# TrondVQ/UncertaintyQuantification-SleepApnea-1DCNN

Hardware: AMD Instinct MI355X
Metric: 30s-windows/sec for MCD T=50 & DE M=8 inference at 1/2/4/8 MI355X (higher is better)
Workload: dtype fp32; 1 GPU; global_batch=16384, seq_len=60, parallelism=dp1, mcd_passes=50, de_members=8, bn_mode_mcd=batch

## Files before the change

uncertaintyquantification_sleepapnea_1dcnn_amd/csrc/x3_dense_map.h:

```cpp
#pragma once

#ifndef __host__
#define APNEAUQ_X3_DENSE_MAP_PLAIN 1
#define __host__
#define __device__
#endif

namespace apneauq {
namespace x3 {
namespace dense {

constexpr int kLen = 60, kSlot = 64, kHaloRows = 4;

__host__ __device__ constexpr long long tiles(long long n_win, int rows) { return (kLen * n_win + rows - 1) / rows; }
__host__ __device__ constexpr int max_windows(int rows) { return (kLen - 4 + rows - 1) / kLen + 1; }
__host__ __device__ constexpr int lds_rows(int rows) { return kHaloRows + kSlot * max_windows(rows) + kHaloRows; }

__host__ __device__ constexpr long long first_row(long long tl, int rows) { return tl * rows; }
__host__ __device__ constexpr int first_window(long long tl, int rows) { return (int)(first_row(tl, rows) / kLen); }
__host__ __device__ constexpr int offset(long long tl, int rows) { return (int)(first_row(tl, rows) % kLen); }
__host__ __device__ constexpr int windows(int off, int rows) { return (off + rows - 1) / kLen + 1; }

__host__ __device__ constexpr int slot_of(int dl) { return (int)(((unsigned)dl & 1023u) * 1093u >> 16); }
__host__ __device__ constexpr int step_of(int dl) { return dl - kLen * slot_of(dl); }
__host__ __device__ constexpr int lds_row(int dl) { return kHaloRows + dl + (kSlot - kLen) * slot_of(dl); }

__host__ __device__ constexpr int staged_units(int rows, int pad) { return rows + 2 * pad; }
__host__ __device__ constexpr bool staged(int dl, int off, int rows, int pad) {
  return dl >= 0 && dl >= off - pad && dl < off + rows + pad && dl < kLen * windows(off, rows);
}

}
}
}

#ifdef APNEAUQ_X3_DENSE_MAP_PLAIN
#undef __host__
#undef __device__
#undef APNEAUQ_X3_DENSE_MAP_PLAIN
#endif
```

uncertaintyquantification_sleepapnea_1dcnn_amd/csrc/x3_layers.hip:

```cpp
#include "common.h"
#include "x3_args.h"
#include "x3_dense_map.h"

namespace apneauq {
namespace x3 {

typedef _Float16 f16x8 __attribute__((ext_vector_type(8)));
typedef _Float16 f16x4 __attribute__((ext_vector_type(4)));
typedef _Float16 f16x2 __attribute__((ext_vector_type(2)));
typedef __attribute__((address_space(1))) const f16x8 gf16x8;

constexpr int kStagers = 4;
constexpr int kL = 60, kSR = 64, kHalo = 4;
__host__ __device__ constexpr int row_bytes(int ck) { return 4 * ck + 32; }
__device__ __forceinline__ int sample_prescale(unsigned rmax_bits, const float* amax) {
  const float b = __builtin_fmaf(amax[0], __uint_as_float(rmax_bits), amax[1]);
  int e = 0;
  if (b > 0.f && b < INFINITY) frexpf(b, &e);
  return min(100, max(-100, 14 - e));
}

__host__ __device__ constexpr int lds_rows(int S) { return kHalo + S * kSR + kHalo; }
__host__ __device__ constexpr int buf_bytes(int S, int ck) { return lds_rows(S) * row_bytes(ck); }
__host__ __device__ constexpr int lds_bytes(int S, int cout, int ck, bool dense_rows = false) {
  return 2 * (dense_rows ? dense::lds_rows(kSR * S) * row_bytes(ck) : buf_bytes(S, ck)) + 2 * cout * 8 + 2 * S * 4;
}

template <typename T>
__device__ __forceinline__ T gld(const void* p) {
  return *(const __attribute__((address_space(1))) T*)(p);
}

__device__ __forceinline__ int opaque_tid() {
  int t = threadIdx.x;
  asm volatile("" : "+v"(t));
  return t;
}

__device__ __forceinline__ f32x4 mfma(const f16x8& a, const f16x8& b, const f32x4& c) {
  return __builtin_amdgcn_mfma_f32_16x16x32_f16(a, b, c, 0, 0, 0);
}

__device__ __forceinline__ void lds_barrier() {
  __builtin_amdgcn_fence(__ATOMIC_RELEASE, "workgroup", "local");
  __builtin_amdgcn_s_barrier();
  __builtin_amdgcn_fence(__ATOMIC_ACQUIRE, "workgroup", "local");
}

__device__ __forceinline__ int xcd_wg() {
  const int nwg = gridDim.x, bid = blockIdx.x;
  const int q = nwg / 8, rem = nwg % 8, xcd = bid % 8;
  return (xcd < rem ? xcd * (q + 1) : rem * (q + 1) + (xcd - rem) * q) + bid / 8;
}

template <int NW, int WPC>
constexpr int waves_per_eu() { return NW * WPC > 8 ? (NW * WPC + 3) / 4 : NW * WPC <= 4 ? 1 : 2; }
constexpr int loaders(int lw) { return lw > 0 ? lw : 0; }
template <int CIN, int COUT, int KS, int S, int WM, int WN, bool LAST, int LW, int CK, int WPC, bool PS, bool DENSE = false>
__global__ __launch_bounds__((WM * WN + loaders(LW)) * 64, (waves_per_eu<WM * WN + loaders(LW), WPC>())) void layer_kernel(
    const LayerArgs A) {
  extern __shared__ __attribute__((aligned(16))) char smem[];
  constexpr int NWM = WM * WN, NW = NWM + loaders(LW), kThreads = NW * 64;
  constexpr int kCK = CK, kRowB = row_bytes(CK), NQ = CK / 32, kQ = CK / 4;
  constexpr int PAD = (KS - 1) / 2, kRows = kSR * S;
  static_assert(!DENSE || (!PS && !LAST), "dense rows: batch-moment blocks 2..5 only");
  constexpr int kS = S, kBufB = DENSE ? dense::lds_rows(kRows) * kRowB : buf_bytes(S, CK);
  constexpr int kValidRows = DENSE ? kRows : S * kL, kUnits = kValidRows * kQ;
  constexpr int SW = LW > 0 ? LW : LW < 0 ? (-LW < NW ? -LW : NW) : (kStagers < NW ? kStagers : NW);
  constexpr int kSBase = LW > 0 ? NWM * 64 : 0;
  constexpr int kST = SW * 64;
  constexpr int kMainU = (kUnits + kST - 1) / kST, kNU = kMainU + (DENSE ? 1 : 0);
  constexpr int kEdgeWaves = (2 * PAD * kQ + 63) / 64;
  static_assert(!DENSE || (kUnits % kST == 0 && kEdgeWaves <= SW), "dense rows: whole staging steps per tile");
  static_assert(kST % kQ == 0 && (CK == 32 || CK == 64), "a staging thread keeps one channel quad");
  constexpr int NCH = CIN / kCK, NCTA = COUT / 16, NCT = NCTA / WN, NRT = 4 * S / WM;
  constexpr int NSTEP = NCH * NQ * KS;
  constexpr int RG = NCT >= 4                        ? 1
                     : (NCT >= 3 && NCT * NRT > 16)    ? 1
                     : NCT == 1                        ? 4
                                                       : 2;
  constexpr bool BDB = NCT * NRT <= 24 && RG < 4;
  static_assert(NRT % RG == 0, "row-tile groups");
  constexpr long long FRAG_STEP = (long long)NCTA * 128;
  static_assert(CIN % kCK == 0 && COUT % 16 == 0, "channel tiling");
  static_assert(NCTA % WN == 0 && (4 * S) % WM == 0, "wave tiling");
  static_assert(NRT % 4 == 0, "whole 64-row sample slots per wave row (epilogue keys, block 6 sums)");
  double* st = reinterpret_cast<double*>(smem + 2 * kBufB);
  float* wsc = reinterpret_cast<float*>(smem + 2 * kBufB + 2 * COUT * 8);

  const int tid = threadIdx.x, lane = tid & 63;
  const int wave = __builtin_amdgcn_readfirstlane(tid >> 6);
  const int wn = wave % WN, wm = (wave / WN) % WM;
  const int ct0 = wn * NCT, rt0 = wm * NRT;
  const int m = lane & 15, h = lane >> 4;
  APNEAUQ_DASSERT(blockDim.x == kThreads);

  for (int i = tid; i < 2 * kBufB / 16; i += kThreads) reinterpret_cast<f32x4*>(smem)[i] = f32x4{0.f, 0.f, 0.f, 0.f};
  for (int i = tid; i < 2 * COUT; i += kThreads) st[i] = 0.0;
  __syncthreads();

  const int wg = xcd_wg();
  const int tpg = DENSE ? (int)dense::tiles(A.n_win, kRows) : (A.n_win + S - 1) / S;
  const int total_tiles = tpg * A.groups;
  const int t_begin = (int)((long long)wg * total_tiles / gridDim.x);
  const int t_end = (int)((long long)(wg + 1) * total_tiles / gridDim.x);
  if (t_begin >= t_end) return;
  const int slot = wg % kStatSlots;

  const bool loader = LW > 0 && wave >= NWM;
  const bool stager = LW > 0 ? loader : wave < SW;
  const bool edge_wave = DENSE && wave >= kSBase / 64 && wave - kSBase / 64 < kEdgeWaves;
  auto dense_unit = [&](int u, int tid, int off, int& dl) -> bool {
    const int r = tid / kQ;
    if (u < kMainU) {
      dl = off + r + (kST / kQ) * u;
      return true;
    }
    dl = r < PAD ? off - PAD + r : off + kRows - PAD + r;
    return edge_wave && r < 2 * PAD && dense::staged(dl, off, kRows, PAD);
  };
  struct Stage {
    f32x4 v[kNU];
    f32x4 a, b;
  };
  Stage s0;
  const bool hash_in = A.thr_in != 0u && !A.sign_in;
  const bool sign_in = A.thr_in != 0u && A.sign_in;
  const bool prescale = PS && A.smax_in != nullptr;
  int key_tile = -1;
  unsigned skeys[kS];
  unsigned skey_tile = 0u;
  static_assert(kS <= 8, "packed per-sample exponents");
  constexpr int kSP = (kS + 3) / 4;
  unsigned sa_pack[kSP];
  auto load_chunk = [&](int tile, int c, Stage& R) {
    const int tid = opaque_tid() - kSBase, q = tid % kQ;
    const int g = tile / tpg;
    const int w0 = (tile - g * tpg) * (DENSE ? kRows : kS);
    const float* af = A.aff_in + (long long)g * A.aff_gstride + c * kCK + 4 * q;
    R.a = gld<f32x4>(af);
    R.b = gld<f32x4>(af + CIN);
#pragma unroll
    for (int u = 0; u < kNU; ++u) {
      const int ri = tid / kQ + (kST / kQ) * u;
      R.v[u] = f32x4{-0.f, -0.f, -0.f, -0.f};
      if constexpr (DENSE) {
        const int wf = w0 / kL, off = w0 - wf * kL;
        int dl;
        if (dense_unit(u, tid, off, dl) && wf + dense::slot_of(dl) < A.n_win) {
          const long long r0 = (A.in_shared ? 0ll : (long long)g * A.n_win * kL) + wf * kL;
          R.v[u] = gld<f32x4>(A.in + (r0 + dl) * CIN + c * kCK + 4 * q);
        }
      } else if (ri < kValidRows) {
        const int s = ri / kL, t = ri - s * kL, w = w0 + s;
        if (w < A.n_win) {
          const long long si = A.in_shared ? w : (long long)g * A.n_win + w;
          R.v[u] = gld<f32x4>(A.in + (si * kL + t) * CIN + c * kCK + 4 * q);
        }
      }
    }
  };
  auto store_chunk = [&](int tile, int c, char* buf, const Stage& R) {
    const int tid = opaque_tid() - kSBase, q = tid % kQ;
    const int g = tile / tpg;
    const int w0 = (tile - g * tpg) * (DENSE ? kRows : kS);
    if (tile != key_tile) {
      const unsigned skey = stream_key(A.seed, A.layer - 1, A.pass_base + g);
      skey_tile = skey;
      const float* am = A.amax_in + (A.aff_gstride ? 2 * g : 0);
      float ws0 = A.wscale[A.p_gstride ? g : 0];
      if (A.gscale_in != nullptr) ws0 *= A.gscale_in[A.aff_gstride ? g : 0];
#pragma unroll
      for (int i = 0; i < kSP; ++i) sa_pack[i] = 0u;
      if (DENSE && tid == 0) wsc[(tile & 1) * kS] = ws0;
#pragma unroll
      for (int s = 0; s < (DENSE ? 0 : kS); ++s) {
        skeys[s] = sample_key(skey, A.window_offset + w0 + s);
        int sa = 0;
        if (prescale && w0 + s < A.n_win) {
          const long long si = A.in_shared ? w0 + s : (long long)g * A.n_win + w0 + s;
          sa = sample_prescale(A.smax_in[si], am);
          sa_pack[s >> 2] |= ((unsigned)sa & 0xFFu) << (8 * (s & 3));
        }
        if (tid == s) wsc[(tile & 1) * kS + s] = ldexpf(ws0, -sa);
      }
      key_tile = tile;
    }
#pragma unroll
    for (int u = 0; u < kNU; ++u) {
      const int ri = tid / kQ + (kST / kQ) * u;
      int s, t, w, lrow;
      if constexpr (DENSE) {
        const int wf = w0 / kL, off = w0 - wf * kL;
        int dl;
        if (!dense_unit(u, tid, off, dl)) continue;
        s = dense::slot_of(dl), t = dl - s * kL, w = wf + s, lrow = dense::lds_row(dl);
      } else {
        if (ri >= kValidRows) continue;
        s = ri / kL, t = ri - s * kL, w = w0 + s, lrow = kHalo + s * kSR + t;
      }
      const f32x4 v = R.v[u];
      bool keep[4];
      if (hash_in) {
        unsigned k;
        if constexpr (!PS) {
          k = sample_key(skey_tile, A.window_offset + w);
        } else {
          k = skeys[0];
#pragma unroll
          for (int j = 1; j < kS; ++j) k = s == j ? skeys[j] : k;
        }
        const unsigned b01 = dropout_bits2(k, t, c * kCK + 4 * q);
        const unsigned b23 = dropout_bits2(k, t, c * kCK + 4 * q + 2);
        keep[0] = (b01 & 0xFFFFu) >= A.thr_in;
        keep[1] = (b01 >> 16) >= A.thr_in;
        keep[2] = (b23 & 0xFFFFu) >= A.thr_in;
        keep[3] = (b23 >> 16) >= A.thr_in;
      } else if (sign_in) {
#pragma unroll
        for (int i = 0; i < 4; ++i) keep[i] = !__builtin_signbit(v[i]);
      } else {
#pragma unroll
        for (int i = 0; i < 4; ++i) keep[i] = true;
      }
      const bool valid = w < A.n_win;
      int sa = 0;
      if (prescale) {
        unsigned sp = sa_pack[0];
#pragma unroll
        for (int i = 1; i < kSP; ++i) sp = (s >> 2) == i ? sa_pack[i] : sp;
        sa = __builtin_amdgcn_sbfe((int)sp, 8 * (s & 3), 8);
      }
      float a[4];
#pragma unroll
      for (int i = 0; i < 4; ++i) a[i] = (valid && keep[i]) ? ldexpf(__builtin_fmaf(v[i], R.a[i], R.b[i]), sa) : 0.f;
      uint2 hi, lo;
#pragma unroll
      for (int p = 0; p < 2; ++p) {
        const unsigned u = __builtin_bit_cast(unsigned, (f16x2){(_Float16)a[2 * p], (_Float16)a[2 * p + 1]});
        unsigned l;
        asm("v_fma_mixlo_f16 %0, %1, -1.0, %2 op_sel_hi:[1,0,0]" : "=v"(l) : "v"(u), "v"(a[2 * p]));
        asm("v_fma_mixhi_f16 %0, %1, -1.0, %2 op_sel:[1,0,0] op_sel_hi:[1,0,0]"
                     : "+v"(l)
                     : "v"(u), "v"(a[2 * p + 1]));
        (p ? hi.y : hi.x) = u;
        (p ? lo.y : lo.x) = l;
      }
      char* row = buf + lrow * kRowB + 8 * q;
      *reinterpret_cast<uint2*>(row) = hi;
      *reinterpret_cast<uint2*>(row + 2 * kCK) = lo;
    }
  };

  f32x4 acc[NCT][NRT];
#pragma unroll
  for (int ct = 0; ct < NCT; ++ct)
#pragma unroll
    for (int rt = 0; rt < NRT; ++rt) acc[ct][rt] = f32x4{0.f, 0.f, 0.f, 0.f};
  auto wbase = [&](int tile) -> const gf16x8* {
    const int g = tile / tpg;
    return (const gf16x8*)(A.wfrag) + (long long)g * A.w_gstride + ct0 * 128 + lane;
  };
  f16x8 ah[NCT], al[NCT];
  auto load_a = [&](const gf16x8* p, f16x8 (&xh)[NCT], f16x8 (&xl)[NCT]) {
#pragma unroll
    for (int ct = 0; ct < NCT; ++ct) {
      xh[ct] = p[ct * 128];
      xl[ct] = p[ct * 128 + 64];
    }
  };

  const int bofs = ((rt0 * 16 + m + kHalo - PAD) * kRowB) + 16 * h;

  auto compute_chunk = [&](int c, int off, const char* buf, const gf16x8* wcur, const gf16x8* wnxt, auto&& hook) {
    const char* bp[DENSE ? NRT : 1];
    if constexpr (DENSE) {
#pragma unroll
      for (int rt = 0; rt < NRT; ++rt)
        bp[rt] = buf + bofs + (off + (dense::kSlot - kL) * ((off + (rt0 + rt) * 16 + m) / kL)) * kRowB;
    }
#pragma unroll
    for (int kk = 0; kk < NQ * KS; ++kk) {
      const int q2 = kk / KS, j = kk - q2 * KS;
      const char* bb = buf + bofs + q2 * 64;
      const int s = c * NQ * KS + kk;
      const gf16x8* np = (s + 1 < NSTEP) ? wcur + (long long)(s + 1) * FRAG_STEP : wnxt;
      f16x8 nh[NCT], nl[NCT];
      load_a(np, nh, nl);
      __builtin_amdgcn_sched_barrier(0);
      auto ldb = [&](int rt, f16x8& h_, f16x8& l_) {
        const char* br = DENSE ? bp[rt] + q2 * 64 : bb;
        h_ = *reinterpret_cast<const f16x8*>(br + (rt * 16 + j) * kRowB);
        l_ = *reinterpret_cast<const f16x8*>(br + (rt * 16 + j) * kRowB + 2 * kCK);
      };
      f16x8 bh[RG], bl[RG];
#pragma unroll
      for (int r = 0; r < RG; ++r) ldb(r, bh[r], bl[r]);
#pragma unroll
      for (int rg = 0; rg < NRT; rg += RG) {
        f16x8 bh2[RG], bl2[RG];
#pragma unroll
        for (int r = 0; r < RG; ++r) {
          bh2[r] = bh[r];
          bl2[r] = bl[r];
          if (BDB && rg + RG < NRT) ldb(rg + RG + r, bh2[r], bl2[r]);
          if (!BDB) ldb(rg + r, bh[r], bl[r]);
        }
        __builtin_amdgcn_sched_barrier(0);
#pragma unroll
        for (int r = 0; r < RG; ++r)
#pragma unroll
          for (int ct = 0; ct < NCT; ++ct) acc[ct][rg + r] = mfma(ah[ct], bh[r], acc[ct][rg + r]);
#pragma unroll
        for (int r = 0; r < RG; ++r)
#pragma unroll
          for (int ct = 0; ct < NCT; ++ct) acc[ct][rg + r] = mfma(al[ct], bh[r], acc[ct][rg + r]);
#pragma unroll
        for (int r = 0; r < RG; ++r)
#pragma unroll
          for (int ct = 0; ct < NCT; ++ct) acc[ct][rg + r] = mfma(ah[ct], bl[r], acc[ct][rg + r]);
#pragma unroll
        for (int r = 0; r < RG; ++r) {
          bh[r] = bh2[r];
          bl[r] = bl2[r];
        }
      }
#pragma unroll
      for (int ct = 0; ct < NCT; ++ct) {
        ah[ct] = nh[ct];
        al[ct] = nl[ct];
      }
      __builtin_amdgcn_sched_barrier(0);
      if (kk == (NQ * KS) / 2) hook();
    }
  };

  auto epilogue = [&](int tile) {
    const int lane = opaque_tid() & 63, m = lane & 15, h = lane >> 4;
    const int g = tile / tpg;
    const int w0 = (tile - g * tpg) * (DENSE ? kRows : kS);
    float wsq[NRT / 4];
#pragma unroll
    for (int q = 0; q < NRT / 4; ++q) wsq[q] = wsc[(tile & 1) * kS + (DENSE ? 0 : (rt0 >> 2) + q)];
    const bool track = PS && !LAST && A.smax_out != nullptr;
    float mxs[NRT / 4];
#pragma unroll
    for (int q = 0; q < NRT / 4; ++q) mxs[q] = 0.f;
    const float* bias = A.bias + (long long)g * A.p_gstride;
    const bool drop = (LAST || A.sign_out) && A.thr_out != 0u;
    constexpr int NKEY = DENSE ? dense::max_windows(kRows) : NRT / 4;
    const int wf = DENSE ? w0 / kL : 0, off = DENSE ? w0 - wf * kL : 0;
    unsigned skeys[NKEY];
    if (drop) {
      const unsigned skey = stream_key(A.seed, A.layer, A.pass_base + g);
#pragma unroll
      for (int q = 0; q < NKEY; ++q)
        skeys[q] = DENSE ? __builtin_amdgcn_readfirstlane(sample_key(skey, A.window_offset + wf + q))
                         : sample_key(skey, A.window_offset + w0 + (rt0 >> 2) + q);
    }
#pragma unroll
    for (int ct = 0; ct < NCT; ++ct) {
      const int co0 = (ct0 + ct) * 16 + 4 * h;
      const f32x4 b4 = gld<f32x4>(bias + co0);
      f32x4 s1 = {0.f, 0.f, 0.f, 0.f}, s2 = s1, k1 = s1, k0 = s1;
      int mo = m;
      if constexpr (DENSE) asm volatile("" : "+v"(mo));
#pragma unroll
      for (int rt = 0; rt < NRT; ++rt) {
        int t, w, sl = 0;
        bool valid;
        if constexpr (DENSE) {
          const int dl = off + (rt0 + rt) * 16 + mo;
          sl = dense::slot_of(dl), w = wf + sl, t = dl - sl * kL, valid = w < A.n_win;
        } else {
          const int s = (rt0 + rt) >> 2;
          t = (((rt0 + rt) & 3) << 4) + m, w = w0 + s, valid = t < kL && w < A.n_win;
        }
        f32x4 r;
#pragma unroll
        for (int e = 0; e < 4; ++e) r[e] = fmaxf(__builtin_fmaf(acc[ct][rt][e], wsq[rt >> 2], b4[e]), 0.f);
        acc[ct][rt] = f32x4{0.f, 0.f, 0.f, 0.f};
        bool keep[4] = {true, true, true, true};
        if (drop) {
          unsigned key = skeys[DENSE ? 0 : rt >> 2];
          if constexpr (DENSE) {
#pragma unroll
            for (int q = 1; q < NKEY; ++q) key = sl == q ? skeys[q] : key;
          }
          const unsigned b01 = dropout_bits2(key, t, co0), b23 = dropout_bits2(key, t, co0 + 2);
          keep[0] = (b01 & 0xFFFFu) >= A.thr_out;
          keep[1] = (b01 >> 16) >= A.thr_out;
          keep[2] = (b23 & 0xFFFFu) >= A.thr_out;
          keep[3] = (b23 >> 16) >= A.thr_out;
        }
        if (valid) {
#pragma unroll
          for (int e = 0; e < 4; ++e) {
            s1[e] += r[e];
            s2[e] = __builtin_fmaf(r[e], r[e], s2[e]);
            if (!LAST) mxs[rt >> 2] = fmaxf(mxs[rt >> 2], r[e]);
            if constexpr (LAST) {
              k1[e] += keep[e] ? r[e] : 0.f;
              k0[e] += keep[e] ? 1.f : 0.f;
            }
          }
          if constexpr (!LAST) {
            const long long sample = (long long)g * A.n_win + w;
            f32x4 o = r;
            if (drop) {
#pragma unroll
              for (int e = 0; e < 4; ++e) o[e] = keep[e] ? r[e] : __builtin_copysignf(r[e], -1.f);
            }
            *reinterpret_cast<f32x4*>(A.out + (sample * kL + t) * COUT + co0) = o;
          }
        }
        if constexpr (LAST) {
          if ((rt & 3) == 3) {
#pragma unroll
            for (int e = 0; e < 4; ++e) {
              k1[e] = group16_sum(k1[e]);
              k0[e] = group16_sum(k0[e]);
            }
            const int wl = w0 + (rt0 + rt) / 4;
            if (m == 0 && wl < A.n_win) {
              float* o = A.out + ((long long)g * A.n_win + wl) * (2 * COUT);
              *reinterpret_cast<f32x4*>(o + co0) = k1;
              *reinterpret_cast<f32x4*>(o + COUT + co0) = k0;
            }
            k1 = f32x4{0.f, 0.f, 0.f, 0.f};
            k0 = k1;
          }
        }
      }
      if (A.stats != nullptr) {
#pragma unroll
        for (int e = 0; e < 4; ++e) {
          const float a = group16_sum(s1[e]), b = group16_sum(s2[e]);
          if (m == 0) {
            atomicAdd(&st[co0 + e], (double)a);
            atomicAdd(&st[COUT + co0 + e], (double)b);
          }
        }
      }
    }
    if (track) {
#pragma unroll
      for (int q = 0; q < NRT / 4; ++q) {
        const float mq = wave_max(mxs[q]);
        const int w = w0 + (rt0 >> 2) + q;
        if (lane == 0 && w < A.n_win) atomicMax(A.smax_out + (long long)g * A.n_win + w, __float_as_uint(mq));
      }
    }
  };

  auto flush_stats = [&](int g) {
    __syncthreads();
    if (A.stats != nullptr) {
      double* dst = A.stats + ((long long)g * kStatSlots + slot) * 2 * COUT;
      for (int i = tid; i < 2 * COUT; i += kThreads) {
        atomicAdd(dst + i, st[i]);
        st[i] = 0.0;
      }
    }
    __syncthreads();
  };

  const int total = (t_end - t_begin) * NCH;
  auto chunk_tile = [&](int it) { return t_begin + it / NCH; };
  auto tile_off = [&](int tile) { return DENSE ? (int)((long long)(tile % tpg) * kRows % kL) : 0; };
  int g_cur = t_begin / tpg;
  if constexpr (LW > 0) {
    if (loader) {
      if (stager) {
        load_chunk(t_begin, 0, s0);
        store_chunk(t_begin, 0, smem, s0);
      }
      lds_barrier();
      if (stager && total > 1) load_chunk(chunk_tile(1), 1 % NCH, s0);
#pragma unroll 1
      for (int it = 0; it < total; ++it) {
        const int tile = chunk_tile(it), c = it - (tile - t_begin) * NCH;
        if (c == 0) {
          const int g = tile / tpg;
          if (g != g_cur) {
            flush_stats(g_cur);
            g_cur = g;
          }
        }
        if (stager && it + 1 < total) store_chunk(chunk_tile(it + 1), (it + 1) % NCH, smem + ((it + 1) & 1) * kBufB, s0);
        lds_barrier();
        if (stager && it + 2 < total) load_chunk(chunk_tile(it + 2), (it + 2) % NCH, s0);
      }
      flush_stats(g_cur);
      return;
    }
    lds_barrier();
    load_a(wbase(t_begin), ah, al);
#pragma unroll 1
    for (int it = 0; it < total; ++it) {
      const int tile = chunk_tile(it), c = it - (tile - t_begin) * NCH;
      if (c == 0) {
        const int g = tile / tpg;
        if (g != g_cur) {
          flush_stats(g_cur);
          g_cur = g;
        }
      }
      const gf16x8* wcur = wbase(tile);
      const gf16x8* wnxt = wbase(tile + 1 < t_end ? tile + 1 : tile);
      compute_chunk(c, tile_off(tile), smem + (it & 1) * kBufB, wcur, wnxt, []() {});
      if (c == NCH - 1) epilogue(tile);
      lds_barrier();
    }
    flush_stats(g_cur);
    return;
  }
  if (stager) {
    load_chunk(t_begin, 0, s0);
    store_chunk(t_begin, 0, smem, s0);
  }
  lds_barrier();
  if (stager && total > 1) load_chunk(chunk_tile(1), 1 % NCH, s0);
  load_a(wbase(t_begin), ah, al);
#pragma unroll 1
  for (int it = 0; it < total; ++it) {
    const int tile = chunk_tile(it), c = it - (tile - t_begin) * NCH;
    if (c == 0) {
      const int g = tile / tpg;
      if (g != g_cur) {
        flush_stats(g_cur);
        g_cur = g;
      }
    }
    const gf16x8* wcur = wbase(tile);
    const gf16x8* wnxt = wbase(tile + 1 < t_end ? tile + 1 : tile);
    char* buf = smem + (it & 1) * kBufB;
    char* nbuf = smem + ((it + 1) & 1) * kBufB;
    compute_chunk(c, tile_off(tile), buf, wcur, wnxt, [&]() {
      if (stager && it + 1 < total) store_chunk(chunk_tile(it + 1), (it + 1) % NCH, nbuf, s0);
    });
    if (c == NCH - 1) epilogue(tile);
    lds_barrier();
    if (stager && it + 2 < total) load_chunk(chunk_tile(it + 2), (it + 2) % NCH, s0);
  }
  flush_stats(g_cur);
}

__global__ __launch_bounds__(256) void l1_kernel(const L1Args A) {
  __shared__ float xs[kL1Win][kL + 6][4];
  __shared__ float red[2][2][128];
  __shared__ unsigned wmax[kL1Win];
  const int g = blockIdx.x / A.blocks_per_group;
  const int w0 = (blockIdx.x - g * A.blocks_per_group) * kL1Win;
  const int tid = threadIdx.x, c = tid & 127, half = tid >> 7;
  for (int i = tid; i < kL1Win * (kL + 6) * 4; i += 256) {
    const int s = i / ((kL + 6) * 4), r = (i / 4) % (kL + 6), ci = i & 3;
    const int t = r - 3, w = w0 + s;
    xs[s][r][ci] = (t >= 0 && t < kL && w < A.n_win) ? A.x[((long long)w * kL + t) * 4 + ci] : 0.f;
  }
  float wr[7][4];
#pragma unroll
  for (int j = 0; j < 7; ++j)
#pragma unroll
    for (int ci = 0; ci < 4; ++ci) wr[j][ci] = A.w[(((long long)g * 7 + j) * 4 + ci) * 128 + c];
  const float bc = A.b[g * 128 + c];
  if (tid < kL1Win) wmax[tid] = 0u;
  __syncthreads();
  float s1 = 0.f, s2 = 0.f;
  for (int s = 0; s < kL1Win; ++s) {
    const int w = w0 + s;
    if (w >= A.n_win) break;
    float* o = A.out + (((long long)g * A.n_win + w) * kL) * 128 + c;
    float mx = 0.f;
    for (int t = half * 30; t < half * 30 + 30; ++t) {
      float v = bc;
#pragma unroll
      for (int j = 0; j < 7; ++j)
#pragma unroll
        for (int ci = 0; ci < 4; ++ci) v = __builtin_fmaf(xs[s][t + j][ci], wr[j][ci], v);
      v = fmaxf(v, 0.f);
      o[t * 128] = v;
      s1 += v;
      s2 = __builtin_fmaf(v, v, s2);
      mx = fmaxf(mx, v);
    }
    if (A.smax != nullptr) {
      mx = wave_max(mx);
      if ((tid & 63) == 0) atomicMax(&wmax[s], __float_as_uint(mx));
    }
  }
  if (A.stats != nullptr || A.smax != nullptr) {
    red[half][0][c] = s1;
    red[half][1][c] = s2;
    __syncthreads();
    if (A.stats != nullptr && tid < 128) {
      double* dst = A.stats + ((long long)g * kStatSlots + (blockIdx.x % kStatSlots)) * 2 * 128;
      atomicAdd(dst + c, (double)red[0][0][c] + (double)red[1][0][c]);
      atomicAdd(dst + 128 + c, (double)red[0][1][c] + (double)red[1][1][c]);
    }
    if (A.smax != nullptr && tid < kL1Win && w0 + tid < A.n_win) A.smax[(long long)g * A.n_win + w0 + tid] = wmax[tid];
  }
}

__device__ __forceinline__ void aff_moments(const AffArgs& A, int g, int c, float& mean, float& var) {
  const double* p = A.stats + (long long)g * kStatSlots * 2 * A.C + c;
  double a = 0.0, b = 0.0;
#pragma unroll
  for (int s = 0; s < kStatSlots; ++s) {
    a += p[s * 2 * A.C];
    b += p[s * 2 * A.C + A.C];
  }
  const double mu = a * A.inv_count;
  mean = (float)mu;
  var = (float)fmax(b * A.inv_count - mu * mu, 0.0);
}

__global__ __launch_bounds__(256) void aff_kernel(const AffArgs A) {
  __shared__ float red[2][4];
  const int tid = threadIdx.x;
  if ((int)blockIdx.x == A.groups) {
    for (int c = tid; c < A.C; c += 256)
      for (int g = 0; g < A.groups; ++g) {
        const long long po = (long long)g * A.p_gstride + c;
        float mean, var;
        aff_moments(A, g, c, mean, var);
        for (int r = 0; r < A.repeat; ++r) {
          A.mmean[po] = A.mmean[po] * A.momentum + mean * (1.f - A.momentum);
          A.mvar[po] = A.mvar[po] * A.momentum + var * (1.f - A.momentum);
        }
      }
    return;
  }
  {
    const int g = blockIdx.x;
    float ms = 0.f, mt = 0.f;
    for (int c = tid; c < A.C; c += 256) {
      const long long po = (long long)g * A.p_gstride + c;
      float mean, var;
      if (A.stats != nullptr && !A.running) {
        aff_moments(A, g, c, mean, var);
      } else {
        mean = A.mmean[po];
        var = A.mvar[po];
      }
      const float sc = A.gamma[po] / sqrtf(var + A.eps);
      const float s_ = sc * A.dsc, t_ = (A.beta[po] - mean * sc) * A.dsc;
      A.aff[((long long)g * 2) * A.C + c] = s_;
      A.aff[((long long)g * 2 + 1) * A.C + c] = t_;
      if (A.gscale != nullptr) {
        const double* p = A.stats + (long long)g * kStatSlots * 2 * A.C + A.C + c;
        double q = 0.0;
        for (int s = 0; s < kStatSlots; ++s) q += p[s * 2 * A.C];
        ms = fmaxf(ms, __builtin_fmaf(fabsf(s_), (float)sqrt(fmax(q, 0.0)) * 1.0001f, fabsf(t_)));
      } else {
        ms = fmaxf(ms, fabsf(s_));
        mt = fmaxf(mt, fabsf(t_));
      }
    }
    if (A.gscale != nullptr) {
      ms = wave_max(ms);
      if ((tid & 63) == 0) red[0][tid >> 6] = ms;
      __syncthreads();
      const float bnd = fmaxf(fmaxf(red[0][0], red[0][1]), fmaxf(red[0][2], red[0][3]));
      int e = 0;
      if (bnd > 0.f && bnd < INFINITY) frexpf(bnd, &e);
      const int sa = min(100, max(-100, 14 - e));
      for (int c = tid; c < A.C; c += 256) {
        float* af = A.aff + (long long)g * 2 * A.C + c;
        af[0] = ldexpf(af[0], sa);
        af[A.C] = ldexpf(af[A.C], sa);
      }
      if (tid == 0) A.gscale[g] = ldexpf(1.f, -sa);
      return;
    }
    if (A.amax == nullptr) return;
    ms = wave_max(ms);
    mt = wave_max(mt);
    if ((tid & 63) == 0) {
      red[0][tid >> 6] = ms;
      red[1][tid >> 6] = mt;
    }
    __syncthreads();
    if (tid == 0) {
      A.amax[2 * g] = fmaxf(fmaxf(red[0][0], red[0][1]), fmaxf(red[0][2], red[0][3]));
      A.amax[2 * g + 1] = fmaxf(fmaxf(red[1][0], red[1][1]), fmaxf(red[1][2], red[1][3]));
    }
  }
}

__global__ __launch_bounds__(256) void head_kernel(const HeadArgs A) {
  const int lane = threadIdx.x & 63;
  const long long sidx = (long long)blockIdx.x * 4 + (threadIdx.x >> 6);
  if (sidx >= A.samples) return;
  const int g = (int)(sidx / A.n_win);
  const float* s = A.sums + sidx * 2 * A.C;
  const float* af = A.aff + (long long)g * A.aff_gstride;
  const float* dw = A.dw + (long long)g * A.p_gstride;
  float v = 0.f;
  for (int c = lane; c < A.C; c += 64) v += dw[c] * __builtin_fmaf(af[c], s[c], af[A.C + c] * s[A.C + c]);
  v = wave_sum(v);
  if (lane == 0) {
    const float logit = v * (1.0f / kL) + A.db[A.p_gstride ? g : 0];
    A.out[sidx] = A.out_logits ? logit : 1.0f / (1.0f + expf(-logit));
  }
}

template <int CIN, int COUT, int KS, int S, int WM, int WN, bool LAST, int LW, int CK, int WPC, bool PS, bool DENSE = false>
hipError_t launch_layer(const LayerArgs& A, int grid, hipStream_t stream) {
  constexpr int lds = lds_bytes(S, COUT, CK, DENSE);
  static_assert(WPC * lds <= 160 * 1024, "LDS of the workgroups sharing a CU");
  auto k = layer_kernel<CIN, COUT, KS, S, WM, WN, LAST, LW, CK, WPC, PS, DENSE>;
  static bool attr = false;
  if (!attr) {
    hipError_t e = hipFuncSetAttribute(reinterpret_cast<const void*>(k), hipFuncAttributeMaxDynamicSharedMemorySize, lds);
    if (e != hipSuccess) return e;
    attr = true;
  }
  hipLaunchKernelGGL(k, dim3(grid), dim3((WM * WN + loaders(LW)) * 64), lds, stream, A);
  return hipGetLastError();
}

template <bool HAVE, int CIN, int COUT, int KS, int S, int WM, int WN, int LW, int CK, int WPC>
hipError_t launch_dense(const LayerArgs& A, int grid, hipStream_t stream) {
  if constexpr (HAVE) {
    return launch_layer<CIN, COUT, KS, S, WM, WN, false, (LW > 0 ? LW : -(WM * WN)), CK, WPC, false, true>(A, grid, stream);
  } else {
    return hipErrorInvalidValue;
  }
}

}

#ifdef APNEAUQ_X3_TABLE
#include APNEAUQ_X3_TABLE
#else
#define APNEAUQ_X3_LAYERS(X)                           \
  X(1, 128, 192, 5, 4, 2, 4, false, -8, 0, 32, 1, true) \
  X(2, 192, 224, 3, 2, 1, 7, false, 4, 4, 64, 1, true)  \
  X(3, 224, 96, 7, 4, 2, 2, false, 4, 4, 32, 1, true)   \
  X(4, 96, 256, 9, 2, 1, 8, false, 4, 4, 32, 1, true)   \
  X(5, 256, 96, 9, 4, 2, 2, true, 4, 4, 64, 1, false)
#endif

int x3_lds_bytes(int layer) {
#define APNEAUQ_X3_LDS(L, CI, CO, K, S, WM, WN, LAST, LW, LWB, CK, WPC, DENSE) \
  if (layer == L) return x3::lds_bytes(S, CO, CK);
  APNEAUQ_X3_LAYERS(APNEAUQ_X3_LDS)
#undef APNEAUQ_X3_LDS
  return 0;
}

int x3_tile_samples(int layer) {
#define APNEAUQ_X3_TS(L, CI, CO, K, S, WM, WN, LAST, LW, LWB, CK, WPC, DENSE) \
  if (layer == L) return S;
  APNEAUQ_X3_LAYERS(APNEAUQ_X3_TS)
#undef APNEAUQ_X3_TS
  return 0;
}

bool x3_has_dense(int layer) {
#define APNEAUQ_X3_HD(L, CI, CO, K, S, WM, WN, LAST, LW, LWB, CK, WPC, DENSE) \
  if (layer == L) return DENSE && !LAST;
  APNEAUQ_X3_LAYERS(APNEAUQ_X3_HD)
#undef APNEAUQ_X3_HD
  return false;
}

int x3_wg_per_cu(int layer) {
#define APNEAUQ_X3_WPC(L, CI, CO, K, S, WM, WN, LAST, LW, LWB, CK, WPC, DENSE) \
  if (layer == L) return WPC;
  APNEAUQ_X3_LAYERS(APNEAUQ_X3_WPC)
#undef APNEAUQ_X3_WPC
  return 1;
}

hipError_t x3_launch_layer(int layer, const x3::LayerArgs& A, int grid, bool dense_rows, hipStream_t stream) {
  using namespace x3;
  const bool ps = A.smax_in != nullptr || A.smax_out != nullptr;
#define APNEAUQ_X3_LAUNCH(L, CI, CO, K, S, WM, WN, LAST, LW, LWB, CK, WPC, DENSE)                                  \
  if (layer == L) {                                                                                       \
    if (dense_rows)                                                                                       \
      return ps ? hipErrorInvalidValue                                                                    \
                : launch_dense<DENSE && !LAST, CI, CO, K, S, WM, WN, LWB, CK, WPC>(A, grid, stream);       \
    return ps ? launch_layer<CI, CO, K, S, WM, WN, LAST, LW, CK, WPC, true>(A, grid, stream)               \
              : launch_layer<CI, CO, K, S, WM, WN, LAST, LWB, CK, WPC, false>(A, grid, stream);            \
  }
  APNEAUQ_X3_LAYERS(APNEAUQ_X3_LAUNCH)
#undef APNEAUQ_X3_LAUNCH
  return hipErrorInvalidValue;
}

hipError_t x3_launch_l1(const x3::L1Args& A, hipStream_t stream) {
  const int grid = A.groups * A.blocks_per_group;
  if (grid <= 0) return hipSuccess;
  hipLaunchKernelGGL(x3::l1_kernel, dim3(grid), dim3(256), 0, stream, A);
  return hipGetLastError();
}

hipError_t x3_launch_aff(const x3::AffArgs& A, hipStream_t stream) {
  const int blocks = A.groups + (A.stats != nullptr && A.update ? 1 : 0);
  hipLaunchKernelGGL(x3::aff_kernel, dim3(blocks), dim3(256), 0, stream, A);
  return hipGetLastError();
}

hipError_t x3_launch_head(const x3::HeadArgs& A, hipStream_t stream) {
  if (A.samples <= 0) return hipSuccess;
  hipLaunchKernelGGL(x3::head_kernel, dim3((A.samples + 3) / 4), dim3(256), 0, stream, A);
  return hipGetLastError();
}

}
```

Before: 64770 windows/s.

## Precompute per-tile dense row descriptors and dropout keys into LDS tables

For the dense-row layer path, each tile's row geometry (LDS row, time step, window slot, validity) and per-row dropout mask words are computed once into double-buffered LDS tables. The next tile's tables are written during the last channel chunk of the current tile. Staging and the epilogue then read these tables instead of recomputing slot divisions and sample hash keys per unit and per row-tile, and output addressing is simplified to a linear row offset. The cost is extra LDS per workgroup and table-write work; occupancy may also drop if LDS becomes the limit.

```diff
diff --git a/uncertaintyquantification_sleepapnea_1dcnn_amd/csrc/x3_dense_map.h b/uncertaintyquantification_sleepapnea_1dcnn_amd/csrc/x3_dense_map.h
--- a/uncertaintyquantification_sleepapnea_1dcnn_amd/csrc/x3_dense_map.h
+++ b/uncertaintyquantification_sleepapnea_1dcnn_amd/csrc/x3_dense_map.h
@@ -30,6 +30,25 @@
   return dl >= 0 && dl >= off - pad && dl < off + rows + pad && dl < kLen * windows(off, rows);
 }
 
+constexpr int kDescStepShift = 9, kDescSlotShift = 15, kDescValidShift = 18;
+__host__ __device__ constexpr unsigned desc_pack(int lrow, int step, int slot, bool valid) {
+  return (unsigned)lrow | (unsigned)step << kDescStepShift | (unsigned)slot << kDescSlotShift |
+         (valid ? 1u : 0u) << kDescValidShift;
+}
+__host__ __device__ constexpr int desc_lds_row(unsigned d) { return (int)(d & 511u); }
+__host__ __device__ constexpr int desc_step(unsigned d) { return (int)(d >> kDescStepShift & 63u); }
+__host__ __device__ constexpr int desc_slot(unsigned d) { return (int)(d >> kDescSlotShift & 7u); }
+__host__ __device__ constexpr bool desc_valid(unsigned d) { return (d >> kDescValidShift & 1u) != 0u; }
+__host__ __device__ constexpr unsigned row_desc(int rel, int off, int rows, int pad, int rows_left) {
+  const int dl = off + rel;
+  if (!staged(dl, off, rows, pad)) return 0u;
+  return desc_pack(lds_row(dl), step_of(dl), slot_of(dl), rel < rows_left);
+}
+__host__ __device__ constexpr unsigned slot_row_desc(int ri, int rows_left) {
+  return desc_pack(lds_row(ri), step_of(ri), slot_of(ri), ri < rows_left);
+}
+__host__ __device__ constexpr unsigned mask_word(unsigned sample_key, int step) { return sample_key ^ ((unsigned)step << 9); }
+
 }
 }
 }
diff --git a/uncertaintyquantification_sleepapnea_1dcnn_amd/csrc/x3_layers.hip b/uncertaintyquantification_sleepapnea_1dcnn_amd/csrc/x3_layers.hip
--- a/uncertaintyquantification_sleepapnea_1dcnn_amd/csrc/x3_layers.hip
+++ b/uncertaintyquantification_sleepapnea_1dcnn_amd/csrc/x3_layers.hip
@@ -22,8 +22,10 @@
 
 __host__ __device__ constexpr int lds_rows(int S) { return kHalo + S * kSR + kHalo; }
 __host__ __device__ constexpr int buf_bytes(int S, int ck) { return lds_rows(S) * row_bytes(ck); }
-__host__ __device__ constexpr int lds_bytes(int S, int cout, int ck, bool dense_rows = false) {
-  return 2 * (dense_rows ? dense::lds_rows(kSR * S) * row_bytes(ck) : buf_bytes(S, ck)) + 2 * cout * 8 + 2 * S * 4;
+__host__ __device__ constexpr int tab_rows(int S, int ks) { return kSR * S + (ks - 1); }
+__host__ __device__ constexpr int lds_bytes(int S, int cout, int ck, int ks, bool dense_rows = false) {
+  return 2 * (dense_rows ? dense::lds_rows(kSR * S) * row_bytes(ck) : buf_bytes(S, ck)) + 2 * cout * 8 + 2 * S * 4 +
+         (dense_rows ? 2 * kSR * S * 4 + 2 * tab_rows(S, ks) * 8 : 0);
 }
 
 template <typename T>
@@ -87,6 +89,10 @@
   static_assert(NRT % 4 == 0, "whole 64-row sample slots per wave row (epilogue keys, block 6 sums)");
   double* st = reinterpret_cast<double*>(smem + 2 * kBufB);
   float* wsc = reinterpret_cast<float*>(smem + 2 * kBufB + 2 * COUT * 8);
+  constexpr int kTabRows = tab_rows(S, KS);
+  static_assert(!DENSE || CIN / CK >= 2, "row tables: a tile's tables are written one chunk of the same workgroup ahead");
+  unsigned* ektab = reinterpret_cast<unsigned*>(smem + 2 * kBufB + 2 * COUT * 8 + 2 * S * 4);
+  uint2* stab = reinterpret_cast<uint2*>(smem + 2 * kBufB + 2 * COUT * 8 + 2 * S * 4 + 2 * kRows * 4);
 
   const int tid = threadIdx.x, lane = tid & 63;
   const int wave = __builtin_amdgcn_readfirstlane(tid >> 6);
@@ -94,10 +100,6 @@
   const int ct0 = wn * NCT, rt0 = wm * NRT;
   const int m = lane & 15, h = lane >> 4;
   APNEAUQ_DASSERT(blockDim.x == kThreads);
-
-  for (int i = tid; i < 2 * kBufB / 16; i += kThreads) reinterpret_cast<f32x4*>(smem)[i] = f32x4{0.f, 0.f, 0.f, 0.f};
-  for (int i = tid; i < 2 * COUT; i += kThreads) st[i] = 0.0;
-  __syncthreads();
 
   const int wg = xcd_wg();
   const int tpg = DENSE ? (int)dense::tiles(A.n_win, kRows) : (A.n_win + S - 1) / S;
@@ -110,14 +112,14 @@
   const bool loader = LW > 0 && wave >= NWM;
   const bool stager = LW > 0 ? loader : wave < SW;
   const bool edge_wave = DENSE && wave >= kSBase / 64 && wave - kSBase / 64 < kEdgeWaves;
-  auto dense_unit = [&](int u, int tid, int off, int& dl) -> bool {
+  auto unit_row = [&](int u, int tid, int& rel) -> bool {
     const int r = tid / kQ;
     if (u < kMainU) {
-      dl = off + r + (kST / kQ) * u;
+      rel = r + (kST / kQ) * u;
       return true;
     }
-    dl = r < PAD ? off - PAD + r : off + kRows - PAD + r;
-    return edge_wave && r < 2 * PAD && dense::staged(dl, off, kRows, PAD);
+    rel = r < PAD ? r - PAD : kRows - PAD + r;
+    return edge_wave && r < 2 * PAD;
   };
   struct Stage {
     f32x4 v[kNU];
@@ -133,29 +135,66 @@
   static_assert(kS <= 8, "packed per-sample exponents");
   constexpr int kSP = (kS + 3) / 4;
   unsigned sa_pack[kSP];
+  struct Geo {
+    int g, w0, wf, off, rows_left;
+  };
+  auto tile_geo = [&](int tile) {
+    Geo G;
+    G.g = tile / tpg;
+    G.w0 = (tile - G.g * tpg) * (DENSE ? kRows : kS);
+    G.wf = DENSE ? G.w0 / kL : G.w0, G.off = DENSE ? G.w0 - G.wf * kL : 0;
+    const long long left = (long long)(A.n_win - G.wf) * kL - G.off;
+    G.rows_left = (int)(left < 1024 ? left : 1024);
+    return G;
+  };
+  const bool mask_out = DENSE && A.sign_out && A.thr_out != 0u;
+  auto write_tables = [&](int tile) {
+    if constexpr (DENSE) {
+      const int tid = opaque_tid() - kSBase;
+      const Geo G = tile_geo(tile);
+      const unsigned ikey = stream_key(A.seed, A.layer - 1, A.pass_base + G.g);
+      const unsigned okey = stream_key(A.seed, A.layer, A.pass_base + G.g);
+#pragma unroll
+      for (int i0 = 0; i0 < kTabRows; i0 += kST) {
+        const int i = i0 + tid, rel = i - PAD;
+        if (i < kTabRows) {
+          const unsigned d = dense::row_desc(rel, G.off, kRows, PAD, G.rows_left);
+          const unsigned win = A.window_offset + G.wf + dense::desc_slot(d);
+          const int t = dense::desc_step(d);
+          stab[(tile & 1) * kTabRows + i] = uint2{d, hash_in ? dense::mask_word(sample_key(ikey, win), t) : 0u};
+          if (mask_out && rel >= 0 && rel < kRows) ektab[(tile & 1) * kRows + rel] = dense::mask_word(sample_key(okey, win), t);
+        }
+      }
+    }
+  };
   auto load_chunk = [&](int tile, int c, Stage& R) {
     const int tid = opaque_tid() - kSBase, q = tid % kQ;
-    const int g = tile / tpg;
-    const int w0 = (tile - g * tpg) * (DENSE ? kRows : kS);
-    const float* af = A.aff_in + (long long)g * A.aff_gstride + c * kCK + 4 * q;
+    const Geo G = tile_geo(tile);
+    const float* af = A.aff_in + (long long)G.g * A.aff_gstride + c * kCK + 4 * q;
     R.a = gld<f32x4>(af);
     R.b = gld<f32x4>(af + CIN);
-#pragma unroll
-    for (int u = 0; u < kNU; ++u) {
-      const int ri = tid / kQ + (kST / kQ) * u;
-      R.v[u] = f32x4{-0.f, -0.f, -0.f, -0.f};
-      if constexpr (DENSE) {
-        const int wf = w0 / kL, off = w0 - wf * kL;
-        int dl;
-        if (dense_unit(u, tid, off, dl) && wf + dense::slot_of(dl) < A.n_win) {
-          const long long r0 = (A.in_shared ? 0ll : (long long)g * A.n_win * kL) + wf * kL;
-          R.v[u] = gld<f32x4>(A.in + (r0 + dl) * CIN + c * kCK + 4 * q);
-        }
-      } else if (ri < kValidRows) {
-        const int s = ri / kL, t = ri - s * kL, w = w0 + s;
-        if (w < A.n_win) {
-          const long long si = A.in_shared ? w : (long long)g * A.n_win + w;
-          R.v[u] = gld<f32x4>(A.in + (si * kL + t) * CIN + c * kCK + 4 * q);
+    if constexpr (DENSE) {
+      const long long row0 = (A.in_shared ? 0ll : (long long)G.g * A.n_win * kL) + G.w0;
+      const float* in = A.in + row0 * CIN + c * kCK + 4 * q;
+#pragma unroll
+      for (int u = 0; u < kNU; ++u) {
+        int rel;
+        bool have = unit_row(u, tid, rel);
+        if (u >= kMainU) have = have && dense::staged(G.off + rel, G.off, kRows, PAD);
+        R.v[u] = f32x4{-0.f, -0.f, -0.f, -0.f};
+        if (have && rel < G.rows_left) R.v[u] = gld<f32x4>(in + rel * CIN);
+      }
+    } else {
+#pragma unroll
+      for (int u = 0; u < kNU; ++u) {
+        const int ri = tid / kQ + (kST / kQ) * u;
+        R.v[u] = f32x4{-0.f, -0.f, -0.f, -0.f};
+        if (ri < kValidRows) {
+          const int s = ri / kL, t = ri - s * kL, w = G.w0 + s;
+          if (w < A.n_win) {
+            const long long si = A.in_shared ? w : (long long)G.g * A.n_win + w;
+            R.v[u] = gld<f32x4>(A.in + (si * kL + t) * CIN + c * kCK + 4 * q);
+          }
         }
       }
     }
@@ -164,6 +203,7 @@
     const int tid = opaque_tid() - kSBase, q = tid % kQ;
     const int g = tile / tpg;
     const int w0 = (tile - g * tpg) * (DENSE ? kRows : kS);
+    if (DENSE && c == NCH - 1 && tile + 1 < t_end) write_tables(tile + 1);
     if (tile != key_tile) {
       const unsigned skey = stream_key(A.seed, A.layer - 1, A.pass_base + g);
       skey_tile = skey;
@@ -186,32 +226,41 @@
       }
       key_tile = tile;
     }
+    const uint2* tab = stab + (tile & 1) * kTabRows + PAD;
 #pragma unroll
     for (int u = 0; u < kNU; ++u) {
-      const int ri = tid / kQ + (kST / kQ) * u;
-      int s, t, w, lrow;
+      int s, lrow;
+      bool valid;
+      unsigned kt = 0u;
       if constexpr (DENSE) {
-        const int wf = w0 / kL, off = w0 - wf * kL;
-        int dl;
-        if (!dense_unit(u, tid, off, dl)) continue;
-        s = dense::slot_of(dl), t = dl - s * kL, w = wf + s, lrow = dense::lds_row(dl);
+        int rel;
+        if (!unit_row(u, tid, rel)) continue;
+        const uint2 e = tab[rel];
+        if (e.x == 0u) continue;
+        s = dense::desc_slot(e.x), lrow = dense::desc_lds_row(e.x), valid = dense::desc_valid(e.x), kt = e.y;
       } else {
+        const int ri = tid / kQ + (kST / kQ) * u;
         if (ri >= kValidRows) continue;
-        s = ri / kL, t = ri - s * kL, w = w0 + s, lrow = kHalo + s * kSR + t;
+        s = ri / kL;
+        const int t = ri - s * kL;
+        lrow = kHalo + s * kSR + t, valid = w0 + s < A.n_win;
+        if (hash_in) {
+          unsigned k;
+          if constexpr (!PS) {
+            k = sample_key(skey_tile, A.window_offset + w0 + s);
+          } else {
+            k = skeys[0];
+#pragma unroll
+            for (int j = 1; j < kS; ++j) k = s == j ? skeys[j] : k;
+          }
+          kt = dense::mask_word(k, t);
+        }
       }
       const f32x4 v = R.v[u];
       bool keep[4];
       if (hash_in) {
-        unsigned k;
-        if constexpr (!PS) {
-          k = sample_key(skey_tile, A.window_offset + w);
-        } else {
-          k = skeys[0];
-#pragma unroll
-          for (int j = 1; j < kS; ++j) k = s == j ? skeys[j] : k;
-        }
-        const unsigned b01 = dropout_bits2(k, t, c * kCK + 4 * q);
-        const unsigned b23 = dropout_bits2(k, t, c * kCK + 4 * q + 2);
+        const unsigned cp = (unsigned)(c * kCK + 4 * q) >> 1;
+        const unsigned b01 = mix32(kt ^ cp), b23 = mix32(kt ^ (cp + 1u));
         keep[0] = (b01 & 0xFFFFu) >= A.thr_in;
         keep[1] = (b01 >> 16) >= A.thr_in;
         keep[2] = (b23 & 0xFFFFu) >= A.thr_in;
@@ -223,7 +272,6 @@
 #pragma unroll
         for (int i = 0; i < 4; ++i) keep[i] = true;
       }
-      const bool valid = w < A.n_win;
       int sa = 0;
       if (prescale) {
         unsigned sp = sa_pack[0];
@@ -348,16 +396,15 @@
     for (int q = 0; q < NRT / 4; ++q) mxs[q] = 0.f;
     const float* bias = A.bias + (long long)g * A.p_gstride;
     const bool drop = (LAST || A.sign_out) && A.thr_out != 0u;
-    constexpr int NKEY = DENSE ? dense::max_windows(kRows) : NRT / 4;
-    const int wf = DENSE ? w0 / kL : 0, off = DENSE ? w0 - wf * kL : 0;
+    constexpr int NKEY = DENSE ? 1 : NRT / 4;
     unsigned skeys[NKEY];
-    if (drop) {
+    if (!DENSE && drop) {
       const unsigned skey = stream_key(A.seed, A.layer, A.pass_base + g);
 #pragma unroll
-      for (int q = 0; q < NKEY; ++q)
-        skeys[q] = DENSE ? __builtin_amdgcn_readfirstlane(sample_key(skey, A.window_offset + wf + q))
-                         : sample_key(skey, A.window_offset + w0 + (rt0 >> 2) + q);
-    }
+      for (int q = 0; q < NKEY; ++q) skeys[q] = sample_key(skey, A.window_offset + w0 + (rt0 >> 2) + q);
+    }
+    const long long left = (long long)A.n_win * kL - w0;
+    const int rows_left = DENSE ? (int)(left < kRows ? left : kRows) : 0;
 #pragma unroll
     for (int ct = 0; ct < NCT; ++ct) {
       const int co0 = (ct0 + ct) * 16 + 4 * h;
@@ -365,13 +412,15 @@
       f32x4 s1 = {0.f, 0.f, 0.f, 0.f}, s2 = s1, k1 = s1, k0 = s1;
       int mo = m;
       if constexpr (DENSE) asm volatile("" : "+v"(mo));
+      const int rel0 = rt0 * 16 + mo;
+      const unsigned* ek = ektab + (tile & 1) * kRows + rel0;
+      float* orow = DENSE ? A.out + (((long long)g * A.n_win * kL + w0 + rel0) * COUT + co0) : nullptr;
 #pragma unroll
       for (int rt = 0; rt < NRT; ++rt) {
-        int t, w, sl = 0;
+        int t = 0, w = 0;
         bool valid;
         if constexpr (DENSE) {
-          const int dl = off + (rt0 + rt) * 16 + mo;
-          sl = dense::slot_of(dl), w = wf + sl, t = dl - sl * kL, valid = w < A.n_win;
+          valid = rel0 + rt * 16 < rows_left;
         } else {
           const int s = (rt0 + rt) >> 2;
           t = (((rt0 + rt) & 3) << 4) + m, w = w0 + s, valid = t < kL && w < A.n_win;
@@ -382,12 +431,13 @@
         acc[ct][rt] = f32x4{0.f, 0.f, 0.f, 0.f};
         bool keep[4] = {true, true, true, true};
         if (drop) {
-          unsigned key = skeys[DENSE ? 0 : rt >> 2];
+          unsigned b01, b23;
           if constexpr (DENSE) {
-#pragma unroll
-            for (int q = 1; q < NKEY; ++q) key = sl == q ? skeys[q] : key;
+            const unsigned kt = ek[rt * 16];
+            b01 = mix32(kt ^ ((unsigned)co0 >> 1)), b23 = mix32(kt ^ (((unsigned)co0 >> 1) + 1u));
+          } else {
+            b01 = dropout_bits2(skeys[rt >> 2], t, co0), b23 = dropout_bits2(skeys[rt >> 2], t, co0 + 2);
           }
-          const unsigned b01 = dropout_bits2(key, t, co0), b23 = dropout_bits2(key, t, co0 + 2);
           keep[0] = (b01 & 0xFFFFu) >= A.thr_out;
           keep[1] = (b01 >> 16) >= A.thr_out;
           keep[2] = (b23 & 0xFFFFu) >= A.thr_out;
@@ -411,7 +461,10 @@
 #pragma unroll
               for (int e = 0; e < 4; ++e) o[e] = keep[e] ? r[e] : __builtin_copysignf(r[e], -1.f);
             }
-            *reinterpret_cast<f32x4*>(A.out + (sample * kL + t) * COUT + co0) = o;
+            if constexpr (DENSE)
+              *reinterpret_cast<f32x4*>(orow + rt * 16 * COUT) = o;
+            else
+              *reinterpret_cast<f32x4*>(A.out + (sample * kL + t) * COUT + co0) = o;
           }
         }
         if constexpr (LAST) {
@@ -457,7 +510,7 @@
     __syncthreads();
     if (A.stats != nullptr) {
       double* dst = A.stats + ((long long)g * kStatSlots + slot) * 2 * COUT;
-      for (int i = tid; i < 2 * COUT; i += kThreads) {
+      for (int i = DENSE ? opaque_tid() : tid; i < 2 * COUT; i += kThreads) {
         atomicAdd(dst + i, st[i]);
         st[i] = 0.0;
       }
@@ -465,6 +518,10 @@
     __syncthreads();
   };
 
+  for (int i = tid; i < 2 * kBufB / 16; i += kThreads) reinterpret_cast<f32x4*>(smem)[i] = f32x4{0.f, 0.f, 0.f, 0.f};
+  for (int i = tid; i < 2 * COUT; i += kThreads) st[i] = 0.0;
+  if (DENSE && stager) write_tables(t_begin);
+  __syncthreads();
   const int total = (t_end - t_begin) * NCH;
   auto chunk_tile = [&](int it) { return t_begin + it / NCH; };
   auto tile_off = [&](int tile) { return DENSE ? (int)((long long)(tile % tpg) * kRows % kL) : 0; };
@@ -707,7 +764,7 @@
 
 template <int CIN, int COUT, int KS, int S, int WM, int WN, bool LAST, int LW, int CK, int WPC, bool PS, bool DENSE = false>
 hipError_t launch_layer(const LayerArgs& A, int grid, hipStream_t stream) {
-  constexpr int lds = lds_bytes(S, COUT, CK, DENSE);
+  constexpr int lds = lds_bytes(S, COUT, CK, KS, DENSE);
   static_assert(WPC * lds <= 160 * 1024, "LDS of the workgroups sharing a CU");
   auto k = layer_kernel<CIN, COUT, KS, S, WM, WN, LAST, LW, CK, WPC, PS, DENSE>;
   static bool attr = false;
@@ -744,7 +801,7 @@
 
 int x3_lds_bytes(int layer) {
 #define APNEAUQ_X3_LDS(L, CI, CO, K, S, WM, WN, LAST, LW, LWB, CK, WPC, DENSE) \
-  if (layer == L) return x3::lds_bytes(S, CO, CK);
+  if (layer == L) return x3::lds_bytes(S, CO, CK, K);
   APNEAUQ_X3_LAYERS(APNEAUQ_X3_LDS)
 #undef APNEAUQ_X3_LDS
   return 0;
```

After: 65900 windows/s, median of 6. +1.7%, better.
